# ronghanghu/vit_10b_fsdp_example

Hardware: AMD Instinct MI355X
Metric: images/sec (whole node) for ViT-10B bs=128 224px --fake_data (higher is better)
Workload: dtype bf16; 1 GPU; model=ViT-10B (5120d/32h/32L, patch14, 224px), global_batch=128, seq_len=256, parallelism=fsdp1, grad_ckpt=True, grad_ckpt_blocks=13, fuse_residual=False, init=device

## Files before the change

csrc/fgemm.hip:

```cpp

#ifndef VITFSDP_KERNELS_ONLY
#include <ATen/cuda/CUDAContext.h>
#include <torch/extension.h>

#include <cstdlib>
#endif

#include "mfma_tiles.h"

namespace {

constexpr int kBM = 256;
constexpr int kBN = 256;
constexpr int kThreads = 512;

template <int BK>
struct FgemmShared {
  static constexpr int SK = BK == 64 ? 64 : BK + 8;
  short a_tile[2][kBM][SK];
  short b_tile[2][kBN][SK];
};

template <int BK>
__device__ __forceinline__ int swz(int row, int col) {
  if (BK == 64) {
    return col ^ ((row & 7) * 8);
  }
  return col ^ (((row >> 3) & 1) * (BK / 2));
}

__device__ __forceinline__ bf16x8 lds_read_b128(unsigned byte_addr) {
  bf16x8 v;
  asm volatile("ds_read_b128 %0, %1 offset:0" : "=v"(v) : "v"(byte_addr));
  return v;
}

template <int EPI, int BK>
__global__ __launch_bounds__(kThreads, BK == 64 ? 1 : 2) void fgemm_abt_kernel(
    const short* __restrict__ a,
    const short* __restrict__ b,
    const short* __restrict__ bias,
    short* __restrict__ c,
    short* __restrict__ aux,
    int M, int N, int K) {
  constexpr bool WITH_BIAS = EPI >= 1;
  constexpr int kSK = FgemmShared<BK>::SK;
  constexpr int kChunks = BK / 32;
  HIP_DYNAMIC_SHARED(char, smem_raw)
  FgemmShared<BK>& sm = *reinterpret_cast<FgemmShared<BK>*>(smem_raw);

  const int tid = threadIdx.x;
  const int lane = tid & 63;
  const int wave = tid >> 6;
  const int col = lane & 15;
  const int seg = lane >> 4;
  const int wm = wave >> 2;
  const int wn = wave & 3;

  int bx = blockIdx.x, by = blockIdx.y;
  {
    const int gx = gridDim.x, gy = gridDim.y;
    const int nwg = gx * gy;
    const int bid = (int)(blockIdx.x + blockIdx.y * gx);
    int sx = 2, sy = 4;
    if (gy % 4 != 0) {
      if (gy % 2 == 0) { sx = 4; sy = 2; }
      else { sx = 8; sy = 1; }
    }
    if ((nwg & 7) == 0 && gx % sx == 0 && gy % sy == 0) {
      const int xcd = bid & 7, cid = bid >> 3;
      const int lw = gx / sx, lh = gy / sy;
      const int gm = (lw % 4 == 0) ? 4 : ((lw % 2 == 0) ? 2 : 1);
      const int per_band = gm * lh;
      const int band = cid / per_band, r = cid % per_band;
      bx = (xcd % sx) * lw + band * gm + (r % gm);
      by = (xcd / sx) * lh + r / gm;
    } else if ((nwg & 7) == 0) {
      const int swz = xcd_swizzle_m_major(bid, nwg);
      bx = swz % gx;
      by = swz / gx;
    }
  }
  const long m0 = (long)bx * kBM;
  const long n0 = (long)by * kBN;

  constexpr int kVecs = kBM * BK / 8 / kThreads;
  constexpr int kPerRow = BK / 8;
  const int s_r0 = tid / kPerRow;
  const int s_c8 = (tid % kPerRow) * 8;
  constexpr int kRowsPerCall = 1024 / (BK * 2);
  constexpr int kCalls = kBM / (8 * kRowsPerCall);
  bf16x8 a_st[BK == 64 ? 1 : kVecs], b_st[BK == 64 ? 1 : kVecs];
  auto issue_dtl = [&](int buf, long k_base) {
    const int l = lane;
    const int rsub = l >> 3;
#pragma unroll
    for (int i = 0; i < kCalls; ++i) {
      const int R = (wave * kCalls + i) * kRowsPerCall;
      const int row = R + rsub;
      const int g = (l & 7) ^ (row & 7);
      __builtin_amdgcn_global_load_lds(
          (const __attribute__((address_space(1))) void*)(
              &a[(m0 + row) * K + k_base + g * 8]),
          (__attribute__((address_space(3))) void*)&sm.a_tile[buf][R][0], 16,
          0, 0);
      __builtin_amdgcn_global_load_lds(
          (const __attribute__((address_space(1))) void*)(
              &b[(n0 + row) * K + k_base + g * 8]),
          (__attribute__((address_space(3))) void*)&sm.b_tile[buf][R][0], 16,
          0, 0);
    }
  };
  auto issue_loads = [&](long k_base) {
    if (BK == 64) return;
#pragma unroll
    for (int i = 0; i < kVecs && BK != 64; ++i) {
      const long row = s_r0 + i * (kThreads / kPerRow);
      a_st[i] =
          *reinterpret_cast<const bf16x8*>(&a[(m0 + row) * K + k_base + s_c8]);
      b_st[i] =
          *reinterpret_cast<const bf16x8*>(&b[(n0 + row) * K + k_base + s_c8]);
    }
  };
  auto write_tiles = [&](int buf) {
    if (BK == 64) return;
#pragma unroll
    for (int i = 0; i < kVecs && BK != 64; ++i) {
      const int row = s_r0 + i * (kThreads / kPerRow);
      const int cc = swz<BK>(row, s_c8);
      *reinterpret_cast<bf16x8*>(&sm.a_tile[buf][row][cc]) = a_st[i];
      *reinterpret_cast<bf16x8*>(&sm.b_tile[buf][row][cc]) = b_st[i];
    }
  };

  f32x4 acc[8][4];
#pragma unroll
  for (int mi = 0; mi < 8; ++mi)
#pragma unroll
    for (int ni = 0; ni < 4; ++ni) acc[mi][ni] = f32x4{0.f, 0.f, 0.f, 0.f};

  const int n_ksteps = K / BK;
  if (BK == 64) {
    issue_dtl(0, 0);
    asm volatile("s_waitcnt vmcnt(0)" ::: "memory");
  } else {
    issue_loads(0);
    write_tiles(0);
  }
  __syncthreads();

  const unsigned lds0 = (unsigned)__builtin_amdgcn_groupstaticsize();
  const unsigned a_base0 = lds0;
  const unsigned b_base0 = lds0 + (unsigned)sizeof(sm.a_tile);
  constexpr unsigned kABufBytes = sizeof(sm.a_tile[0]);
  constexpr unsigned kBBufBytes = sizeof(sm.b_tile[0]);

  for (int ks = 0; ks < n_ksteps; ++ks) {
    const int buf = ks & 1;
    const unsigned a_base = a_base0 + (unsigned)buf * kABufBytes;
    const unsigned b_base = b_base0 + (unsigned)buf * kBBufBytes;
#pragma unroll
    for (int kc = 0; kc < kChunks; ++kc) {
      if (BK == 64) {
        if (kc == 0 && ks + 1 < n_ksteps) issue_dtl(buf ^ 1, (long)(ks + 1) * BK);
      } else if (kc == kChunks - 1 && ks + 1 < n_ksteps) {
        issue_loads((long)(ks + 1) * BK);
      }
      const int kcol = kc * 32 + seg * 8;
      bf16x8 bf[4];
#pragma unroll
      for (int ni = 0; ni < 4; ++ni) {
        const int br = wn * 64 + ni * 16 + col;
        bf[ni] = lds_read_b128(
            b_base + 2u * ((unsigned)(br * kSK + swz<BK>(br, kcol))));
      }
      bf16x8 af[8];
#pragma unroll
      for (int mi = 0; mi < 8; ++mi) {
        const int ar = wm * 128 + mi * 16 + col;
        af[mi] = lds_read_b128(
            a_base + 2u * ((unsigned)(ar * kSK + swz<BK>(ar, kcol))));
      }
      asm volatile("s_waitcnt lgkmcnt(0)"
                   : "+v"(af[0]), "+v"(af[1]), "+v"(af[2]), "+v"(af[3]),
                     "+v"(af[4]), "+v"(af[5]), "+v"(af[6]), "+v"(af[7]),
                     "+v"(bf[0]), "+v"(bf[1]), "+v"(bf[2]), "+v"(bf[3])
                   :
                   : "memory");
      __builtin_amdgcn_s_setprio(1);
#pragma unroll
      for (int mi = 0; mi < 8; ++mi) {
#pragma unroll
        for (int ni = 0; ni < 4; ++ni) {
          acc[mi][ni] = __builtin_amdgcn_mfma_f32_16x16x32_bf16(
              af[mi], bf[ni], acc[mi][ni], 0, 0, 0);
        }
      }
      __builtin_amdgcn_s_setprio(0);
    }
    if (BK == 64) {
      if (ks + 1 < n_ksteps)
        asm volatile("s_waitcnt vmcnt(0)" ::: "memory");
    } else if (ks + 1 < n_ksteps) {
      write_tiles(buf ^ 1);
    }
    __syncthreads();
  }

  float bias_v[4];
  if (WITH_BIAS) {
#pragma unroll
    for (int ni = 0; ni < 4; ++ni) {
      bias_v[ni] = bf16_to_f32(
          (unsigned short)bias[n0 + wn * 64 + ni * 16 + col]);
    }
  }
#pragma unroll
  for (int mi = 0; mi < 8; ++mi) {
#pragma unroll
    for (int r = 0; r < 4; ++r) {
      const long m = m0 + wm * 128 + mi * 16 + seg * 4 + r;
#pragma unroll
      for (int ni = 0; ni < 4; ++ni) {
        const long n = n0 + wn * 64 + ni * 16 + col;
        float v = acc[mi][ni][r];
        if (WITH_BIAS) v += bias_v[ni];
        if (EPI == 2) {
          aux[m * N + n] = (short)f32_to_bf16(v);
          v = 0.5f * v * (1.f + erff(v * 0.70710678118654752f));
        }
        c[m * N + n] = (short)f32_to_bf16(v);
      }
    }
  }
}

template <int EPI>
__global__ __launch_bounds__(kThreads, 1) void fgemm_abt_mi32_kernel(
    const short* __restrict__ a, const short* __restrict__ b,
    const short* __restrict__ bias, short* __restrict__ c,
    short* __restrict__ aux, int M, int N, int K) {
  constexpr bool WITH_BIAS = EPI >= 1;
  constexpr int BK = 64;
  HIP_DYNAMIC_SHARED(char, smem_raw)
  FgemmShared<BK>& sm = *reinterpret_cast<FgemmShared<BK>*>(smem_raw);

  const int tid = threadIdx.x;
  const int lane = tid & 63;
  const int wave = tid >> 6;
  const int l31 = lane & 31;
  const int kseg = lane >> 5;
  const int wm = wave >> 2;
  const int wn = wave & 3;

  int bx = blockIdx.x, by = blockIdx.y;
  {
    const int gx = gridDim.x, gy = gridDim.y;
    const int nwg = gx * gy;
    const int bid = (int)(blockIdx.x + blockIdx.y * gx);
    int sx = 2, sy = 4;
    if (gy % 4 != 0) {
      if (gy % 2 == 0) { sx = 4; sy = 2; }
      else { sx = 8; sy = 1; }
    }
    if ((nwg & 7) == 0 && gx % sx == 0 && gy % sy == 0) {
      const int xcd = bid & 7, cid = bid >> 3;
      const int lw = gx / sx, lh = gy / sy;
      const int gm = (lw % 4 == 0) ? 4 : ((lw % 2 == 0) ? 2 : 1);
      const int per_band = gm * lh;
      const int band = cid / per_band, r = cid % per_band;
      bx = (xcd % sx) * lw + band * gm + (r % gm);
      by = (xcd / sx) * lh + r / gm;
    } else if ((nwg & 7) == 0) {
      const int swzb = xcd_swizzle_m_major(bid, nwg);
      bx = swzb % gx;
      by = swzb / gx;
    }
  }
  const long m0 = (long)bx * kBM;
  const long n0 = (long)by * kBN;

  auto issue_dtl = [&](int buf, long k_base) {
    const int rsub = lane >> 3;
#pragma unroll
    for (int i = 0; i < 4; ++i) {
      const int R = (wave * 4 + i) * 8;
      const int row = R + rsub;
      const int g = (lane & 7) ^ (row & 7);
      __builtin_amdgcn_global_load_lds(
          (const __attribute__((address_space(1))) void*)(
              &a[(m0 + row) * K + k_base + g * 8]),
          (__attribute__((address_space(3))) void*)&sm.a_tile[buf][R][0], 16,
          0, 0);
      __builtin_amdgcn_global_load_lds(
          (const __attribute__((address_space(1))) void*)(
              &b[(n0 + row) * K + k_base + g * 8]),
          (__attribute__((address_space(3))) void*)&sm.b_tile[buf][R][0], 16,
          0, 0);
    }
  };

  f32x16 acc[4][2];
#pragma unroll
  for (int mi = 0; mi < 4; ++mi)
#pragma unroll
    for (int ni = 0; ni < 2; ++ni) acc[mi][ni] = f32x16{};

  const int n_ksteps = K / BK;
  issue_dtl(0, 0);
  asm volatile("s_waitcnt vmcnt(0)" ::: "memory");
  __syncthreads();

  for (int ks = 0; ks < n_ksteps; ++ks) {
    const int buf = ks & 1;
    if (ks + 1 < n_ksteps) issue_dtl(buf ^ 1, (long)(ks + 1) * BK);
#pragma unroll
    for (int kc = 0; kc < 4; ++kc) {
      const int kcol = kc * 16 + kseg * 8;
      bf16x8 bf[2];
#pragma unroll
      for (int ni = 0; ni < 2; ++ni) {
        const int br = wn * 64 + ni * 32 + l31;
        bf[ni] = *reinterpret_cast<const bf16x8*>(
            &sm.b_tile[buf][br][swz<BK>(br, kcol)]);
      }
      __builtin_amdgcn_s_setprio(1);
#pragma unroll
      for (int mi = 0; mi < 4; ++mi) {
        const int ar = wm * 128 + mi * 32 + l31;
        const bf16x8 af = *reinterpret_cast<const bf16x8*>(
            &sm.a_tile[buf][ar][swz<BK>(ar, kcol)]);
#pragma unroll
        for (int ni = 0; ni < 2; ++ni) {
          acc[mi][ni] = __builtin_amdgcn_mfma_f32_32x32x16_bf16(
              af, bf[ni], acc[mi][ni], 0, 0, 0);
        }
      }
      __builtin_amdgcn_s_setprio(0);
    }
    if (ks + 1 < n_ksteps)
      asm volatile("s_waitcnt vmcnt(0)" ::: "memory");
    __syncthreads();
  }

  float bias_v[2];
  if (WITH_BIAS) {
#pragma unroll
    for (int ni = 0; ni < 2; ++ni) {
      bias_v[ni] = bf16_to_f32(
          (unsigned short)bias[n0 + wn * 64 + ni * 32 + l31]);
    }
  }
#pragma unroll
  for (int mi = 0; mi < 4; ++mi) {
#pragma unroll
    for (int g = 0; g < 4; ++g) {
#pragma unroll
      for (int r = 0; r < 4; ++r) {
        const long m = m0 + wm * 128 + mi * 32 + kseg * 4 + g * 8 + r;
#pragma unroll
        for (int ni = 0; ni < 2; ++ni) {
          const long n = n0 + wn * 64 + ni * 32 + l31;
          float v = acc[mi][ni][g * 4 + r];
          if (WITH_BIAS) v += bias_v[ni];
          if (EPI == 2) {
            aux[m * N + n] = (short)f32_to_bf16(v);
            v = 0.5f * v * (1.f + erff(v * 0.70710678118654752f));
          }
          c[m * N + n] = (short)f32_to_bf16(v);
        }
      }
    }
  }
}

#ifdef VITFSDP_KERNELS_ONLY
template __global__ void fgemm_abt_kernel<0, 64>(const short*, const short*,
                                                 const short*, short*, short*,
                                                 int, int, int);
template __global__ void fgemm_abt_kernel<1, 64>(const short*, const short*,
                                                 const short*, short*, short*,
                                                 int, int, int);
template __global__ void fgemm_abt_kernel<2, 64>(const short*, const short*,
                                                 const short*, short*, short*,
                                                 int, int, int);
template __global__ void fgemm_abt_kernel<0, 32>(const short*, const short*,
                                                 const short*, short*, short*,
                                                 int, int, int);
template __global__ void fgemm_abt_mi32_kernel<0>(const short*, const short*,
                                                  const short*, short*,
                                                  short*, int, int, int);
#endif

}

#ifndef VITFSDP_KERNELS_ONLY
namespace {

int fgemm_bk() {
  static int bk = [] {
    const char* e = std::getenv("VITFSDP_FGEMM_BK");
    return (e != nullptr && std::atoi(e) == 32) ? 32 : 64;
  }();
  return bk;
}

int fgemm_mi() {
  static int mi = [] {
    const char* e = std::getenv("VITFSDP_FGEMM_MI");
    return (e != nullptr && std::atoi(e) == 32) ? 32 : 16;
  }();
  return mi;
}

template <int EPI, int BK>
void launch_fgemm(const short* x, const short* w, const short* bias, short* c,
                  short* aux, long M, long N, long K, hipStream_t stream) {
  static bool attr_set = [] {
    (void)hipFuncSetAttribute(
        reinterpret_cast<const void*>(&fgemm_abt_kernel<EPI, BK>),
        hipFuncAttributeMaxDynamicSharedMemorySize, sizeof(FgemmShared<BK>));
    return true;
  }();
  (void)attr_set;
  dim3 grid((unsigned)(M / kBM), (unsigned)(N / kBN));
  hipLaunchKernelGGL((fgemm_abt_kernel<EPI, BK>), grid, dim3(kThreads),
                     sizeof(FgemmShared<BK>), stream, x, w, bias, c, aux,
                     (int)M, (int)N, (int)K);
}

template <int EPI>
void launch_fgemm_mi32(const short* x, const short* w, const short* bias,
                       short* c, short* aux, long M, long N, long K,
                       hipStream_t stream) {
  static bool attr_set = [] {
    (void)hipFuncSetAttribute(
        reinterpret_cast<const void*>(&fgemm_abt_mi32_kernel<EPI>),
        hipFuncAttributeMaxDynamicSharedMemorySize, sizeof(FgemmShared<64>));
    return true;
  }();
  (void)attr_set;
  dim3 grid((unsigned)(M / kBM), (unsigned)(N / kBN));
  hipLaunchKernelGGL((fgemm_abt_mi32_kernel<EPI>), grid, dim3(kThreads),
                     sizeof(FgemmShared<64>), stream, x, w, bias, c, aux,
                     (int)M, (int)N, (int)K);
}

template <int EPI>
void launch_fgemm_bk(const short* x, const short* w, const short* bias,
                     short* c, short* aux, long M, long N, long K,
                     hipStream_t stream) {
  if (fgemm_bk() == 32 && K % 32 == 0)
    launch_fgemm<EPI, 32>(x, w, bias, c, aux, M, N, K, stream);
  else if (fgemm_mi() == 32)
    launch_fgemm_mi32<EPI>(x, w, bias, c, aux, M, N, K, stream);
  else
    launch_fgemm<EPI, 64>(x, w, bias, c, aux, M, N, K, stream);
}

}

torch::Tensor fwd_gemm(torch::Tensor x, torch::Tensor w,
                       c10::optional<torch::Tensor> bias) {
  TORCH_CHECK(x.is_cuda() && x.is_contiguous() && w.is_contiguous(),
              "fwd_gemm: contiguous CUDA tensors required");
  TORCH_CHECK(x.scalar_type() == torch::kBFloat16 &&
              w.scalar_type() == torch::kBFloat16, "fwd_gemm: bf16 only");
  TORCH_CHECK(x.dim() == 2 && w.dim() == 2 && x.size(1) == w.size(1),
              "fwd_gemm: x[M,K], w[N,K] expected");
  const long M = x.size(0), K = x.size(1), N = w.size(0);
  TORCH_CHECK(M % kBM == 0 && N % kBN == 0 && K % 64 == 0,
              "fwd_gemm: needs M%256==0, N%256==0, K%64==0 (got ", M, ",", N,
              ",", K, ")");
  auto c = torch::empty({M, N}, x.options());
  const short* bias_ptr = nullptr;
  torch::Tensor bias_c;
  if (bias.has_value()) {
    bias_c = bias->contiguous();
    TORCH_CHECK(bias_c.scalar_type() == torch::kBFloat16 &&
                bias_c.numel() == N, "fwd_gemm: bias must be bf16 [N]");
    bias_ptr = (const short*)bias_c.data_ptr();
  }
  auto stream = at::cuda::getCurrentCUDAStream();
  if (bias_ptr) {
    launch_fgemm_bk<1>((const short*)x.data_ptr(), (const short*)w.data_ptr(),
                       bias_ptr, (short*)c.data_ptr(), nullptr, M, N, K,
                       stream);
  } else {
    launch_fgemm_bk<0>((const short*)x.data_ptr(), (const short*)w.data_ptr(),
                       nullptr, (short*)c.data_ptr(), nullptr, M, N, K,
                       stream);
  }
  HIP_CHECK_LAST();
  return c;
}

std::vector<torch::Tensor> fwd_gemm_gelu(torch::Tensor x, torch::Tensor w,
                                         torch::Tensor bias) {
  TORCH_CHECK(x.is_cuda() && x.is_contiguous() && w.is_contiguous() &&
              bias.is_contiguous(), "fwd_gemm_gelu: contiguous CUDA only");
  TORCH_CHECK(x.scalar_type() == torch::kBFloat16 &&
              w.scalar_type() == torch::kBFloat16 &&
              bias.scalar_type() == torch::kBFloat16,
              "fwd_gemm_gelu: bf16 only");
  TORCH_CHECK(x.dim() == 2 && w.dim() == 2 && x.size(1) == w.size(1) &&
              bias.numel() == w.size(0), "fwd_gemm_gelu: x[M,K], w[N,K]");
  const long M = x.size(0), K = x.size(1), N = w.size(0);
  TORCH_CHECK(M % kBM == 0 && N % kBN == 0 && K % 64 == 0,
              "fwd_gemm_gelu: needs M%256==0, N%256==0, K%64==0");
  auto c = torch::empty({M, N}, x.options());
  auto aux = torch::empty({M, N}, x.options());
  auto stream = at::cuda::getCurrentCUDAStream();
  launch_fgemm_bk<2>((const short*)x.data_ptr(), (const short*)w.data_ptr(),
                     (const short*)bias.data_ptr(), (short*)c.data_ptr(),
                     (short*)aux.data_ptr(), M, N, K, stream);
  HIP_CHECK_LAST();
  return {c, aux};
}
#endif
```

csrc/mfma_tiles.h:

```cpp
#pragma once

#include "common.h"

typedef __attribute__((ext_vector_type(8))) short bf16x8;
typedef __attribute__((ext_vector_type(4))) float f32x4;
typedef __attribute__((ext_vector_type(16))) float f32x16;
typedef __attribute__((ext_vector_type(2))) unsigned int u32x2;


__device__ __forceinline__ u32x2 tr16_read(unsigned lds_byte_addr) {
  u32x2 v;
  asm volatile("ds_read_b64_tr_b16 %0, %1 offset:0"
               : "=v"(v)
               : "v"(lds_byte_addr));
  return v;
}

template <int N>
__device__ __forceinline__ void lds_wait(u32x2& lo, u32x2& hi) {
  asm volatile("s_waitcnt lgkmcnt(%[cnt])"
               : "+v"(lo), "+v"(hi)
               : [cnt] "i"(N)
               : "memory");
}

__device__ __forceinline__ bf16x8 frag_from(u32x2 lo, u32x2 hi) {
  union {
    u32x2 uu[2];
    bf16x8 v;
  } cv;
  cv.uu[0] = lo;
  cv.uu[1] = hi;
  return cv.v;
}

__device__ __forceinline__ unsigned pack_bf16x2(float lo, float hi) {
  return (unsigned)f32_to_bf16(lo) | ((unsigned)f32_to_bf16(hi) << 16);
}

template <int NC, int STRIDE>
__device__ __forceinline__ void mfma_tr_ring(bf16x8 a, unsigned lds_base,
                                             int seg, int col,
                                             f32x4 (&acc)[NC]) {
  const unsigned lane_base =
      lds_base +
      2u * (unsigned)((seg * 8 + (col >> 2)) * STRIDE + (col & 3) * 4);
  u32x2 bf[2][2];
#pragma unroll
  for (int h = 0; h < 2; ++h)
    bf[0][h] = tr16_read(lane_base + 2u * (4 * h * STRIDE));
#pragma unroll
  for (int c = 0; c < NC; ++c) {
    const int cur = c & 1;
    if (c + 1 < NC) {
#pragma unroll
      for (int h = 0; h < 2; ++h)
        bf[cur ^ 1][h] =
            tr16_read(lane_base + 2u * (4 * h * STRIDE + (c + 1) * 16));
      lds_wait<2>(bf[cur][0], bf[cur][1]);
    } else {
      lds_wait<0>(bf[cur][0], bf[cur][1]);
    }
    acc[c] = __builtin_amdgcn_mfma_f32_16x16x32_bf16(
        a, frag_from(bf[cur][0], bf[cur][1]), acc[c], 0, 0, 0);
  }
}

__device__ __forceinline__ bf16x8 c_to_a_layout(const unsigned (&pk)[2][2],
                                                int seg, int col) {
  union {
    unsigned u[4];
    bf16x8 v;
  } cvt;
#pragma unroll
  for (int j2 = 0; j2 < 4; ++j2) {
    const int src = col + 16 * ((seg & 1) * 2 + (j2 >> 1));
    const unsigned lo = (unsigned)__shfl((int)pk[0][j2 & 1], src);
    const unsigned hi = (unsigned)__shfl((int)pk[1][j2 & 1], src);
    cvt.u[j2] = (seg >> 1) ? hi : lo;
  }
  return cvt.v;
}

template <int NKC, int D>
__device__ __forceinline__ void load_row_frags(const short* __restrict__ p,
                                               bool valid, int seg,
                                               bf16x8 (&frag)[NKC]) {
#pragma unroll
  for (int kc = 0; kc < NKC; ++kc) {
    const int d0 = kc * 32 + seg * 8;
    if (valid && d0 + 8 <= D) {
      frag[kc] = *reinterpret_cast<const bf16x8*>(&p[d0]);
    } else {
#pragma unroll
      for (int j = 0; j < 8; ++j)
        frag[kc][j] = (valid && d0 + j < D) ? p[d0 + j] : (short)0;
    }
  }
}

template <int ROWS, int COLS, int D, int THREADS>
struct TileStage {
  static constexpr int VPR = COLS / 8;
  static constexpr int N = (ROWS * VPR + THREADS - 1) / THREADS;
  int r[N], c[N];
  __device__ __forceinline__ TileStage() {
#pragma unroll
    for (int i = 0; i < N; ++i) {
      const int idx = (int)threadIdx.x + i * THREADS;
      r[i] = idx / VPR;
      c[i] = (idx % VPR) * 8;
    }
  }
  template <int M>
  __device__ __forceinline__ void load(const short* __restrict__ p,
                                       long row_stride, int row0, int T,
                                       bf16x8 (&st)[M]) const {
#pragma unroll
    for (int i = 0; i < N; ++i) {
      bf16x8 val = {0, 0, 0, 0, 0, 0, 0, 0};
      const int row = row0 + r[i];
      if (r[i] < ROWS && row < T && (COLS <= D || c[i] < D)) {
        val = *reinterpret_cast<const bf16x8*>(
            &p[(long)row * row_stride + c[i]]);
      }
      st[i] = val;
    }
  }
  template <int STRIDE, int M>
  __device__ __forceinline__ void store(short (*tile)[STRIDE],
                                        const bf16x8 (&st)[M]) const {
#pragma unroll
    for (int i = 0; i < N; ++i) {
      if (r[i] < ROWS) {
        *reinterpret_cast<bf16x8*>(&tile[r[i]][c[i]]) = st[i];
      }
    }
  }
};

__device__ __forceinline__ int xcd_swizzle_m_major(int bid, int nwg) {
  return (bid & 7) * (nwg >> 3) + (bid >> 3);
}
```

csrc/wgemm.hip:

```cpp

#ifndef VITFSDP_KERNELS_ONLY
#include <ATen/cuda/CUDAContext.h>
#include <torch/extension.h>
#endif

#include "mfma_tiles.h"

namespace {

constexpr int kBM = 256;
constexpr int kBN = 256;
constexpr int kBK = 64;
constexpr int kThreads = 512;
constexpr int kSA = kBM + 16;
constexpr int kSB = kBN + 16;

struct WgemmShared {
  short a_tile[2][kBK][kSA];
  short b_tile[2][kBK][kSB];
};

__device__ __forceinline__ u32x2 tr_read(unsigned lds_byte_base, int lane15,
                                         int row_base, int col_base,
                                         int row_stride) {
  return tr16_read(lds_byte_base +
                   2u * ((unsigned)((row_base + (lane15 >> 2)) * row_stride +
                                    col_base + (lane15 & 3) * 4)));
}

template <bool WITH_BIAS>
__global__ __launch_bounds__(kThreads, 2) void wgemm_atb_kernel(
    const short* __restrict__ a,
    const short* __restrict__ b,
    short* __restrict__ c,
    float* __restrict__ dbias,
    int K, int M, int N) {
  HIP_DYNAMIC_SHARED(char, smem_raw)
  WgemmShared& sm = *reinterpret_cast<WgemmShared*>(smem_raw);
  const unsigned a_base0 = (unsigned)__builtin_amdgcn_groupstaticsize();
  const unsigned b_base0 = a_base0 + sizeof(sm.a_tile);
  constexpr unsigned kABufBytes = sizeof(sm.a_tile[0]);
  constexpr unsigned kBBufBytes = sizeof(sm.b_tile[0]);

  const int tid = threadIdx.x;
  const int lane = tid & 63;
  const int wave = tid >> 6;
  const int col = lane & 15;
  const int seg = lane >> 4;
  const int wm = wave >> 2;
  const int wn = wave & 3;

  int bx = blockIdx.x, by = blockIdx.y;
  {
    const int nwg = gridDim.x * gridDim.y;
    if ((nwg & 7) == 0) {
      const int swz = xcd_swizzle_m_major(
          (int)(blockIdx.x + blockIdx.y * gridDim.x), nwg);
      bx = swz % gridDim.x;
      by = swz / gridDim.x;
    }
  }
  const long m0 = (long)bx * kBM;
  const long n0 = (long)by * kBN;

  constexpr int kVecs = kBK * (kBM / 8) / kThreads;
  const int s_kr0 = tid >> 5;
  const int s_c8 = (tid & 31) * 8;
  bf16x8 a_st[kVecs], b_st[kVecs];
  auto issue_loads = [&](long k_base) {
#pragma unroll
    for (int i = 0; i < kVecs; ++i) {
      const long krow = k_base + s_kr0 + i * 16;
      a_st[i] = *reinterpret_cast<const bf16x8*>(&a[krow * M + m0 + s_c8]);
      b_st[i] = *reinterpret_cast<const bf16x8*>(&b[krow * N + n0 + s_c8]);
    }
  };
  auto write_tiles = [&](int buf) {
#pragma unroll
    for (int i = 0; i < kVecs; ++i) {
      const int kr = s_kr0 + i * 16;
      *reinterpret_cast<bf16x8*>(&sm.a_tile[buf][kr][s_c8]) = a_st[i];
      *reinterpret_cast<bf16x8*>(&sm.b_tile[buf][kr][s_c8]) = b_st[i];
    }
  };

  f32x4 acc[8][4];
#pragma unroll
  for (int mi = 0; mi < 8; ++mi)
#pragma unroll
    for (int ni = 0; ni < 4; ++ni) acc[mi][ni] = f32x4{0.f, 0.f, 0.f, 0.f};

  float bias_acc[WITH_BIAS ? 8 : 1];
#pragma unroll
  for (int mi = 0; mi < (WITH_BIAS ? 8 : 1); ++mi) bias_acc[mi] = 0.f;

  const int n_ksteps = K / kBK;
  issue_loads(0);
  write_tiles(0);
  __syncthreads();

  for (int ks = 0; ks < n_ksteps; ++ks) {
    const int buf = ks & 1;
    const unsigned a_base = a_base0 + (unsigned)buf * kABufBytes;
    const unsigned b_base = b_base0 + (unsigned)buf * kBBufBytes;
#pragma unroll
    for (int kc = 0; kc < 2; ++kc) {
      if (kc == 1 && ks + 1 < n_ksteps) issue_loads((long)(ks + 1) * kBK);
      u32x2 bf[4][2];
#pragma unroll
      for (int ni = 0; ni < 4; ++ni) {
#pragma unroll
        for (int h = 0; h < 2; ++h) {
          bf[ni][h] = tr_read(b_base, col, kc * 32 + seg * 8 + 4 * h,
                              wn * 64 + ni * 16, kSB);
        }
      }
      u32x2 af[2][2];
#pragma unroll
      for (int h = 0; h < 2; ++h) {
        af[0][h] = tr_read(a_base, col, kc * 32 + seg * 8 + 4 * h,
                           wm * 128 + 0 * 16, kSA);
      }
#pragma unroll
      for (int mi = 0; mi < 8; ++mi) {
        const int cur = mi & 1;
        if (mi < 7) {
#pragma unroll
          for (int h = 0; h < 2; ++h) {
            af[cur ^ 1][h] =
                tr_read(a_base, col, kc * 32 + seg * 8 + 4 * h,
                        wm * 128 + (mi + 1) * 16, kSA);
          }
        }
        if (mi == 0) {
          asm volatile("s_waitcnt lgkmcnt(%[cnt])"
                       : "+v"(af[cur][0]), "+v"(af[cur][1]),
                         "+v"(bf[0][0]), "+v"(bf[0][1]), "+v"(bf[1][0]),
                         "+v"(bf[1][1]), "+v"(bf[2][0]), "+v"(bf[2][1])
                       : [cnt] "i"(2)
                       : "memory");
          asm volatile("" : "+v"(bf[3][0]), "+v"(bf[3][1]));
        } else if (mi < 7) {
          lds_wait<2>(af[cur][0], af[cur][1]);
        } else {
          lds_wait<0>(af[cur][0], af[cur][1]);
        }
        const bf16x8 a_frag = frag_from(af[cur][0], af[cur][1]);
        __builtin_amdgcn_s_setprio(1);
#pragma unroll
        for (int ni = 0; ni < 4; ++ni) {
          acc[mi][ni] = __builtin_amdgcn_mfma_f32_16x16x32_bf16(
              a_frag, frag_from(bf[ni][0], bf[ni][1]), acc[mi][ni], 0, 0, 0);
        }
        __builtin_amdgcn_s_setprio(0);
        if (WITH_BIAS && wn == 0) {
#pragma unroll
          for (int h = 0; h < 2; ++h) {
            bias_acc[mi] +=
                bf16_to_f32((unsigned short)(af[cur][h][0] & 0xffff)) +
                bf16_to_f32((unsigned short)(af[cur][h][0] >> 16)) +
                bf16_to_f32((unsigned short)(af[cur][h][1] & 0xffff)) +
                bf16_to_f32((unsigned short)(af[cur][h][1] >> 16));
          }
        }
      }
    }

    if (ks + 1 < n_ksteps) write_tiles(buf ^ 1);
    __syncthreads();
  }

#pragma unroll
  for (int mi = 0; mi < 8; ++mi) {
#pragma unroll
    for (int r = 0; r < 4; ++r) {
      const long m = m0 + wm * 128 + mi * 16 + seg * 4 + r;
#pragma unroll
      for (int ni = 0; ni < 4; ++ni) {
        const long n = n0 + wn * 64 + ni * 16 + col;
        c[m * N + n] = (short)f32_to_bf16(acc[mi][ni][r]);
      }
    }
    if (WITH_BIAS && wn == 0) {
      float v = bias_acc[mi];
      v += __shfl_xor(v, 16);
      v += __shfl_xor(v, 32);
      if (seg == 0) {
        atomicAdd(&dbias[m0 + wm * 128 + mi * 16 + col], v);
      }
    }
  }
}

#ifdef VITFSDP_KERNELS_ONLY
template __global__ void wgemm_atb_kernel<false>(const short*, const short*,
                                                 short*, float*, int, int,
                                                 int);
#endif

}

#ifndef VITFSDP_KERNELS_ONLY
std::vector<torch::Tensor> wgrad_gemm(torch::Tensor a, torch::Tensor b,
                                      bool with_bias) {
  TORCH_CHECK(a.is_cuda() && a.is_contiguous() && b.is_contiguous());
  TORCH_CHECK(a.scalar_type() == torch::kBFloat16 &&
              b.scalar_type() == torch::kBFloat16);
  TORCH_CHECK(a.dim() == 2 && b.dim() == 2 && a.size(0) == b.size(0));
  const long K = a.size(0), M = a.size(1), N = b.size(1);
  TORCH_CHECK(K % kBK == 0 && M % kBM == 0 && N % kBN == 0,
              "wgrad_gemm: needs K%64==0, M%256==0, N%256==0 (got ", K, ",",
              M, ",", N, ")");
  auto c = torch::empty({M, N}, a.options());
  torch::Tensor dbias;
  float* dbias_ptr = nullptr;
  if (with_bias) {
    dbias = torch::zeros({M}, a.options().dtype(torch::kFloat32));
    dbias_ptr = dbias.data_ptr<float>();
  }
  static bool attr_set = [] {
    hipFuncSetAttribute(
        reinterpret_cast<const void*>(&wgemm_atb_kernel<false>),
        hipFuncAttributeMaxDynamicSharedMemorySize, sizeof(WgemmShared));
    hipFuncSetAttribute(
        reinterpret_cast<const void*>(&wgemm_atb_kernel<true>),
        hipFuncAttributeMaxDynamicSharedMemorySize, sizeof(WgemmShared));
    return true;
  }();
  (void)attr_set;
  dim3 grid((unsigned)(M / kBM), (unsigned)(N / kBN));
  auto stream = at::cuda::getCurrentCUDAStream();
  if (with_bias) {
    hipLaunchKernelGGL(wgemm_atb_kernel<true>, grid, dim3(kThreads),
                       sizeof(WgemmShared), stream,
                       (const short*)a.data_ptr(), (const short*)b.data_ptr(),
                       (short*)c.data_ptr(), dbias_ptr, (int)K, (int)M,
                       (int)N);
  } else {
    hipLaunchKernelGGL(wgemm_atb_kernel<false>, grid, dim3(kThreads),
                       sizeof(WgemmShared), stream,
                       (const short*)a.data_ptr(), (const short*)b.data_ptr(),
                       (short*)c.data_ptr(), nullptr, (int)K, (int)M,
                       (int)N);
  }
  HIP_CHECK_LAST();
  if (with_bias) return {c, dbias};
  return {c};
}
#endif
```

vit_10b_fsdp_example_amd/ops/linear.py:

```python

import contextlib
import os

import torch
import torch.nn as nn
import torch.nn.functional as F
from torch.utils._python_dispatch import TorchDispatchMode

from ._extension import ext, use_hip
from ..tuning import lt_algo_table


_WGRAD_MODE = os.environ.get("VITFSDP_NATIVE_WGRAD", "0")
_NATIVE_WGRAD = _WGRAD_MODE == "1"
_NATIVE_WGRAD_DISPATCH = _WGRAD_MODE == "2"


def _use_native_wgrad(dy2, x2, w):
    if not _NATIVE_WGRAD:
        return False
    if not (dy2.is_cuda and dy2.dtype == torch.bfloat16):
        return False
    m, n = w.shape[0], w.shape[1]
    k = dy2.shape[0]
    if not (k % 64 == 0 and m % 256 == 0 and n % 256 == 0):
        return False
    if m > 16384 or n > 8192:
        return False
    return use_hip(dy2) and hasattr(ext(), "wgrad_gemm")


class _NativeLinearFn(torch.autograd.Function):
    @staticmethod
    def forward(ctx, x, weight, bias):
        ctx.save_for_backward(x, weight)
        ctx.has_bias = bias is not None
        return F.linear(x, weight, bias)

    @staticmethod
    def backward(ctx, dy):
        x, weight = ctx.saved_tensors
        dy2 = dy.reshape(-1, dy.shape[-1])
        x2 = x.reshape(-1, x.shape[-1])
        dx = torch.matmul(dy, weight)

        if _use_native_wgrad(dy2, x2, weight):
            (dw,) = ext().wgrad_gemm(dy2.contiguous(), x2.contiguous(), False)
            db = dy2.sum(0) if ctx.has_bias else None
        else:
            dw = torch.matmul(dy2.t(), x2)
            db = dy2.sum(0) if ctx.has_bias else None
        return dx, dw, db


_MIN_TILES = int(os.environ.get("VITFSDP_WGRAD_MIN_TILES", "256"))


def _wgrad_mm_shapes_ok(m, n, k):
    return (k % 64 == 0 and m % 256 == 0 and n % 256 == 0
            and m <= 16384 and n <= 16384
            and (m // 256) * (n // 256) >= _MIN_TILES)


def _is_wgrad_mm(at, b):
    if at.dim() != 2 or b.dim() != 2 or at.shape[1] != b.shape[0]:
        return False
    m, k = at.shape
    if m < 2 or k < 2:
        return False
    if not (at.stride(0) == 1 and at.stride(1) == m):
        return False
    if not (b.stride(1) == 1 and b.stride(0) == b.shape[1]):
        return False
    return _wgrad_mm_shapes_ok(m, b.shape[1], k)


class NativeWgradMode(TorchDispatchMode):

    def __init__(self, handler=None):
        super().__init__()
        self.hits = 0
        self._handler = handler

    def _route(self, at, b):
        if self._handler is not None:
            return self._handler(at.t(), b)
        (dw,) = ext().wgrad_gemm(at.t().contiguous(), b.contiguous(), False)
        return dw

    def __torch_dispatch__(self, func, types, args=(), kwargs=None):
        kwargs = kwargs or {}
        if (
            func is torch.ops.aten.mm.default
            and _is_wgrad_mm(*args)
            and (
                self._handler is not None
                or (
                    args[0].is_cuda
                    and args[0].dtype == torch.bfloat16
                    and args[1].dtype == torch.bfloat16
                    and use_hip(args[0])
                    and hasattr(ext(), "wgrad_gemm")
                )
            )
        ):
            self.hits += 1
            return self._route(*args)
        return func(*args, **kwargs)


def _op_layout(t):
    if t.dim() != 2:
        return None
    r, c = t.shape
    s0, s1 = t.stride()
    if s1 == 1 and (s0 == c or r == 1):
        return "N"
    if s0 == 1 and (s1 == r or c == 1):
        return "T"
    return None


def _dual_key(a, b):
    la, lb = _op_layout(a), _op_layout(b)
    if la is None or lb is None:
        return None
    return (lb, la, b.shape[1], a.shape[0], a.shape[1])



_GELU_CFG = {"d": 0, "hid": 0}

_FGEMM_MIN_TILES = int(os.environ.get("VITFSDP_FGEMM_MIN_TILES", "256"))


def configure_gelu_fusion(embed_dim, hidden_dim):
    if embed_dim != hidden_dim:
        _GELU_CFG["d"] = int(embed_dim)
        _GELU_CFG["hid"] = int(hidden_dim)


def _gelu_fusion_on():
    return (
        os.environ.get("VITFSDP_FUSED_GELU", "0") == "1"
        and _GELU_CFG["hid"] > 0
    )




def _dgelu_dbias_on():
    return (
        os.environ.get("VITFSDP_FUSED_DGELU_DBIAS", "1") != "0"
        and _GELU_CFG["hid"] > 0
    )



class TunedGemmMode(TorchDispatchMode):

    def __init__(self, table=None, native_wgrad=None, handler=None,
                 dgelu_handler=None):
        super().__init__()
        self.table = lt_algo_table() if table is None else table
        self.native_wgrad = (
            _NATIVE_WGRAD_DISPATCH if native_wgrad is None else native_wgrad
        )
        self._handler = handler
        self.hits = 0
        self.wgrad_hits = 0
        self.fused_gelu = _gelu_fusion_on()
        self._pending_gelu = {}
        self.gelu_hits = 0
        self._dgelu_handler = dgelu_handler
        self.fused_dgelu = _dgelu_dbias_on() and (
            dgelu_handler is not None or self._handler is None
        )
        self._dgelu_stash = None
        self.dgelu_hits = 0
        self.dbias_hits = 0

    def __exit__(self, exc_type, exc_val, exc_tb):
        self._dgelu_stash = None
        return super().__exit__(exc_type, exc_val, exc_tb)

    def _tuned_index(self, a, b):
        if not self.table:
            return None
        key = _dual_key(a, b)
        if key is None:
            return None
        return self.table.get(key)

    def _gpu_ok(self, t):
        if self._handler is not None:
            return True
        return t.is_cuda and t.dtype == torch.bfloat16 and use_hip(t)

    def _route(self, a, b, idx, bias=None):
        if self._handler is not None:
            return self._handler(a, b, idx, bias)
        return ext().lt_gemm(a, b, idx, bias)


    def _is_fc1_fwd(self, key):
        if not (
            key is not None
            and key[0] == "T" and key[1] == "N"
            and key[2] == _GELU_CFG["hid"] and key[4] == _GELU_CFG["d"]
        ):
            return False
        if self._handler is not None:
            return True
        hid, tok = key[2], key[3]
        return (
            tok % 256 == 0 and hid % 256 == 0 and key[4] % 64 == 0
            and (tok // 256) * (hid // 256) >= _FGEMM_MIN_TILES
        )

    def _fused_fc1_fwd(self, a, b, bias):
        if self._handler is not None:
            out, pre = self._handler(a, b, "gelu", bias)
        else:
            out, pre = ext().fwd_gemm_gelu(
                a.contiguous(), b.t().contiguous(), bias
            )
        self.gelu_hits += 1
        if len(self._pending_gelu) > 4:
            self._pending_gelu.clear()
        self._pending_gelu[pre.data_ptr()] = (pre, out)
        return pre


    def _is_mlp_dgelu(self, args, kwargs):
        if len(args) != 2 or kwargs.get("approximate", "none") != "none":
            return False
        dy, x = args
        if not (
            dy.dim() >= 2
            and dy.shape[-1] == _GELU_CFG["hid"]
            and dy.shape == x.shape
            and dy.is_contiguous() and x.is_contiguous()
        ):
            return False
        if self._dgelu_handler is not None:
            return True
        return (
            dy.is_cuda and dy.dtype == torch.bfloat16
            and x.dtype == torch.bfloat16
            and dy.shape[-1] % 8 == 0
            and use_hip(dy)
        )

    def _fused_dgelu(self, dy, x):
        if self._dgelu_handler is not None:
            dx, colsum = self._dgelu_handler(dy, x)
        else:
            dx, colsum = ext().gelu_bwd_colsum(dy, x)
        self.dgelu_hits += 1
        self._dgelu_stash = (dx, colsum)
        return dx

    def _stashed_dbias(self, args, kwargs):
        if self._dgelu_stash is None or kwargs.get("dtype") is not None:
            return None
        dx, colsum = self._dgelu_stash
        t = args[0]
        dims = args[1] if len(args) > 1 else None
        keepdim = args[2] if len(args) > 2 else kwargs.get("keepdim", False)
        if not (
            isinstance(t, torch.Tensor)
            and dims is not None
            and t.dtype == dx.dtype
            and t.device == dx.device
            and t.untyped_storage().data_ptr()
            == dx.untyped_storage().data_ptr()
            and t.storage_offset() == dx.storage_offset()
            and t.numel() == dx.numel()
            and t.dim() >= 2
            and t.shape[-1] == dx.shape[-1]
            and t.is_contiguous()
            and sorted(d % t.dim() for d in dims) == list(range(t.dim() - 1))
        ):
            return None
        self._dgelu_stash = None
        self.dbias_hits += 1
        if keepdim:
            return colsum.view([1] * (t.dim() - 1) + [t.shape[-1]])
        return colsum

    def __torch_dispatch__(self, func, types, args=(), kwargs=None):
        kwargs = kwargs or {}
        if func is torch.ops.aten.mm.default and self._gpu_ok(args[0]):
            a, b = args
            if (
                self.native_wgrad
                and self._handler is None
                and _is_wgrad_mm(a, b)
                and hasattr(ext(), "wgrad_gemm")
            ):
                self.wgrad_hits += 1
                (dw,) = ext().wgrad_gemm(a.t().contiguous(), b.contiguous(),
                                         False)
                return dw
            idx = self._tuned_index(a, b)
            if idx is not None:
                self.hits += 1
                return self._route(a, b, idx)
        elif (
            func is torch.ops.aten.addmm.default
            and len(args) == 3
            and kwargs.get("beta", 1) == 1
            and kwargs.get("alpha", 1) == 1
            and self._gpu_ok(args[1])
            and args[0].dim() == 1
        ):
            bias, a, b = args
            key = _dual_key(a, b)
            if (
                self.fused_gelu
                and self._is_fc1_fwd(key)
                and (self._handler is not None
                     or hasattr(ext(), "fwd_gemm_gelu"))
            ):
                return self._fused_fc1_fwd(a, b, bias)
            idx = self.table.get(key) if (self.table and key) else None
            if idx is not None:
                self.hits += 1
                return self._route(a, b, idx, bias)
        elif self.fused_gelu and func is torch.ops.aten.gelu.default:
            _, out = self._pending_gelu.pop(args[0].data_ptr(), (None, None))
            if out is not None and out.shape == args[0].shape:
                return out
        elif self.fused_dgelu and func is torch.ops.aten.gelu_backward.default:
            if self._is_mlp_dgelu(args, kwargs):
                return self._fused_dgelu(*args)
        elif (
            self._dgelu_stash is not None
            and func is torch.ops.aten.sum.dim_IntList
        ):
            out = self._stashed_dbias(args, kwargs)
            if out is not None:
                return out
        return func(*args, **kwargs)


def gemm_dispatch_context():
    if lt_algo_table() or _gelu_fusion_on() or _dgelu_dbias_on():
        return TunedGemmMode()
    if _NATIVE_WGRAD_DISPATCH:
        return NativeWgradMode()
    return contextlib.nullcontext()


def wgrad_backward_context():
    return gemm_dispatch_context()


class NativeLinear(nn.Linear):

    def forward(self, x):
        if _NATIVE_WGRAD:
            return _NativeLinearFn.apply(x, self.weight, self.bias)
        return F.linear(x, self.weight, self.bias)
```

Before: 65.60 images/sec.

## Rework wgrad GEMM with direct-to-LDS loads, XOR swizzle, and enable it by default

Rewrites the native weight-gradient GEMM so tiles are loaded straight from global memory into LDS via global_load_lds, replacing the register staging and LDS write-back. LDS tiles lose their padding and use an XOR chunk swizzle instead, with precomputed per-lane offsets and immediate-offset transposed reads. The kernel also adopts the shared XCD-clustered tile mapping, now factored into a helper, and launch bounds drop to one block per CU. The default VITFSDP_NATIVE_WGRAD mode becomes dispatch mode 2, so this kernel replaces the library wgrad path, which risks being slower than hipBLASLt for some shapes.

New measurement: 66.26 images/sec (median of 6 runs). +1.0%, better.

```diff
diff --git a/csrc/fgemm.hip b/csrc/fgemm.hip
--- a/csrc/fgemm.hip
+++ b/csrc/fgemm.hip
@@ -57,30 +57,8 @@
   const int wm = wave >> 2;
   const int wn = wave & 3;
 
-  int bx = blockIdx.x, by = blockIdx.y;
-  {
-    const int gx = gridDim.x, gy = gridDim.y;
-    const int nwg = gx * gy;
-    const int bid = (int)(blockIdx.x + blockIdx.y * gx);
-    int sx = 2, sy = 4;
-    if (gy % 4 != 0) {
-      if (gy % 2 == 0) { sx = 4; sy = 2; }
-      else { sx = 8; sy = 1; }
-    }
-    if ((nwg & 7) == 0 && gx % sx == 0 && gy % sy == 0) {
-      const int xcd = bid & 7, cid = bid >> 3;
-      const int lw = gx / sx, lh = gy / sy;
-      const int gm = (lw % 4 == 0) ? 4 : ((lw % 2 == 0) ? 2 : 1);
-      const int per_band = gm * lh;
-      const int band = cid / per_band, r = cid % per_band;
-      bx = (xcd % sx) * lw + band * gm + (r % gm);
-      by = (xcd / sx) * lh + r / gm;
-    } else if ((nwg & 7) == 0) {
-      const int swz = xcd_swizzle_m_major(bid, nwg);
-      bx = swz % gx;
-      by = swz / gx;
-    }
-  }
+  int bx, by;
+  xcd_cluster_tile(bx, by);
   const long m0 = (long)bx * kBM;
   const long n0 = (long)by * kBN;
 
@@ -253,30 +231,8 @@
   const int wm = wave >> 2;
   const int wn = wave & 3;
 
-  int bx = blockIdx.x, by = blockIdx.y;
-  {
-    const int gx = gridDim.x, gy = gridDim.y;
-    const int nwg = gx * gy;
-    const int bid = (int)(blockIdx.x + blockIdx.y * gx);
-    int sx = 2, sy = 4;
-    if (gy % 4 != 0) {
-      if (gy % 2 == 0) { sx = 4; sy = 2; }
-      else { sx = 8; sy = 1; }
-    }
-    if ((nwg & 7) == 0 && gx % sx == 0 && gy % sy == 0) {
-      const int xcd = bid & 7, cid = bid >> 3;
-      const int lw = gx / sx, lh = gy / sy;
-      const int gm = (lw % 4 == 0) ? 4 : ((lw % 2 == 0) ? 2 : 1);
-      const int per_band = gm * lh;
-      const int band = cid / per_band, r = cid % per_band;
-      bx = (xcd % sx) * lw + band * gm + (r % gm);
-      by = (xcd / sx) * lh + r / gm;
-    } else if ((nwg & 7) == 0) {
-      const int swzb = xcd_swizzle_m_major(bid, nwg);
-      bx = swzb % gx;
-      by = swzb / gx;
-    }
-  }
+  int bx, by;
+  xcd_cluster_tile(bx, by);
   const long m0 = (long)bx * kBM;
   const long n0 = (long)by * kBN;
 
diff --git a/csrc/mfma_tiles.h b/csrc/mfma_tiles.h
--- a/csrc/mfma_tiles.h
+++ b/csrc/mfma_tiles.h
@@ -13,6 +13,16 @@
   asm volatile("ds_read_b64_tr_b16 %0, %1 offset:0"
                : "=v"(v)
                : "v"(lds_byte_addr));
+  return v;
+}
+
+template <int OFF>
+__device__ __forceinline__ u32x2 tr16_read_at(unsigned lds_byte_addr) {
+  static_assert(OFF >= 0 && OFF < 65536, "ds offset field is 16 bits");
+  u32x2 v;
+  asm volatile("ds_read_b64_tr_b16 %0, %1 offset:%2"
+               : "=v"(v)
+               : "v"(lds_byte_addr), "n"(OFF));
   return v;
 }
 
@@ -142,3 +152,29 @@
 __device__ __forceinline__ int xcd_swizzle_m_major(int bid, int nwg) {
   return (bid & 7) * (nwg >> 3) + (bid >> 3);
 }
+
+__device__ __forceinline__ void xcd_cluster_tile(int& bx, int& by) {
+  bx = blockIdx.x;
+  by = blockIdx.y;
+  const int gx = gridDim.x, gy = gridDim.y;
+  const int nwg = gx * gy;
+  const int bid = (int)(blockIdx.x + blockIdx.y * gx);
+  int sx = 2, sy = 4;
+  if (gy % 4 != 0) {
+    if (gy % 2 == 0) { sx = 4; sy = 2; }
+    else { sx = 8; sy = 1; }
+  }
+  if ((nwg & 7) == 0 && gx % sx == 0 && gy % sy == 0) {
+    const int xcd = bid & 7, cid = bid >> 3;
+    const int lw = gx / sx, lh = gy / sy;
+    const int gm = (lw % 4 == 0) ? 4 : ((lw % 2 == 0) ? 2 : 1);
+    const int per_band = gm * lh;
+    const int band = cid / per_band, r = cid % per_band;
+    bx = (xcd % sx) * lw + band * gm + (r % gm);
+    by = (xcd / sx) * lh + r / gm;
+  } else if ((nwg & 7) == 0) {
+    const int swz = xcd_swizzle_m_major(bid, nwg);
+    bx = swz % gx;
+    by = swz / gx;
+  }
+}
diff --git a/csrc/wgemm.hip b/csrc/wgemm.hip
--- a/csrc/wgemm.hip
+++ b/csrc/wgemm.hip
@@ -12,24 +12,26 @@
 constexpr int kBN = 256;
 constexpr int kBK = 64;
 constexpr int kThreads = 512;
-constexpr int kSA = kBM + 16;
-constexpr int kSB = kBN + 16;
+static_assert(kBM == kBN, "one staging/read scheme serves both tiles");
+constexpr int kRowBytes = kBM * 2;
 
 struct WgemmShared {
-  short a_tile[2][kBK][kSA];
-  short b_tile[2][kBK][kSB];
+  short a_tile[2][kBK][kBM];
+  short b_tile[2][kBK][kBN];
 };
 
-__device__ __forceinline__ u32x2 tr_read(unsigned lds_byte_base, int lane15,
-                                         int row_base, int col_base,
-                                         int row_stride) {
-  return tr16_read(lds_byte_base +
-                   2u * ((unsigned)((row_base + (lane15 >> 2)) * row_stride +
-                                    col_base + (lane15 & 3) * 4)));
+__device__ __forceinline__ int chunk_xor(int k) {
+  return (k & 3) | (((k >> 3) & 1) << 2);
+}
+
+__device__ __forceinline__ void glds16(const short* gsrc, short* lds_dst) {
+  __builtin_amdgcn_global_load_lds(
+      (const __attribute__((address_space(1))) void*)gsrc,
+      (__attribute__((address_space(3))) void*)lds_dst, 16, 0, 0);
 }
 
 template <bool WITH_BIAS>
-__global__ __launch_bounds__(kThreads, 2) void wgemm_atb_kernel(
+__global__ __launch_bounds__(kThreads, 1) void wgemm_atb_kernel(
     const short* __restrict__ a,
     const short* __restrict__ b,
     short* __restrict__ c,
@@ -50,39 +52,35 @@
   const int wm = wave >> 2;
   const int wn = wave & 3;
 
-  int bx = blockIdx.x, by = blockIdx.y;
-  {
-    const int nwg = gridDim.x * gridDim.y;
-    if ((nwg & 7) == 0) {
-      const int swz = xcd_swizzle_m_major(
-          (int)(blockIdx.x + blockIdx.y * gridDim.x), nwg);
-      bx = swz % gridDim.x;
-      by = swz / gridDim.x;
-    }
-  }
+  int bx, by;
+  xcd_cluster_tile(bx, by);
   const long m0 = (long)bx * kBM;
   const long n0 = (long)by * kBN;
 
-  constexpr int kVecs = kBK * (kBM / 8) / kThreads;
-  const int s_kr0 = tid >> 5;
-  const int s_c8 = (tid & 31) * 8;
-  bf16x8 a_st[kVecs], b_st[kVecs];
-  auto issue_loads = [&](long k_base) {
-#pragma unroll
-    for (int i = 0; i < kVecs; ++i) {
-      const long krow = k_base + s_kr0 + i * 16;
-      a_st[i] = *reinterpret_cast<const bf16x8*>(&a[krow * M + m0 + s_c8]);
-      b_st[i] = *reinterpret_cast<const bf16x8*>(&b[krow * N + n0 + s_c8]);
+  constexpr int kCalls = kBK / 2 / (kThreads / 64);
+  auto issue_dtl = [&](int buf, long k_base) {
+    const int rsub = lane >> 5;
+    const int gl = lane & 31;
+#pragma unroll
+    for (int i = 0; i < kCalls; ++i) {
+      const int R = (wave * kCalls + i) * 2;
+      const int k = R + rsub;
+      const int g = (((gl >> 1) ^ chunk_xor(k)) << 1) | (gl & 1);
+      glds16(&a[(k_base + k) * M + m0 + g * 8], &sm.a_tile[buf][R][0]);
+      glds16(&b[(k_base + k) * N + n0 + g * 8], &sm.b_tile[buf][R][0]);
     }
   };
-  auto write_tiles = [&](int buf) {
-#pragma unroll
-    for (int i = 0; i < kVecs; ++i) {
-      const int kr = s_kr0 + i * 16;
-      *reinterpret_cast<bf16x8*>(&sm.a_tile[buf][kr][s_c8]) = a_st[i];
-      *reinterpret_cast<bf16x8*>(&sm.b_tile[buf][kr][s_c8]) = b_st[i];
-    }
-  };
+
+  const int xr = (col >> 2) | ((seg & 1) << 2);
+  const unsigned lane_off =
+      (unsigned)((seg * 8 + (col >> 2)) * kRowBytes + (col & 3) * 8);
+  unsigned a_off[8], b_off[4];
+#pragma unroll
+  for (int mi = 0; mi < 8; ++mi)
+    a_off[mi] = lane_off + ((unsigned)((wm * 8 + mi) ^ xr) << 5);
+#pragma unroll
+  for (int ni = 0; ni < 4; ++ni)
+    b_off[ni] = lane_off + ((unsigned)((wn * 4 + ni) ^ xr) << 5);
 
   f32x4 acc[8][4];
 #pragma unroll
@@ -95,43 +93,35 @@
   for (int mi = 0; mi < (WITH_BIAS ? 8 : 1); ++mi) bias_acc[mi] = 0.f;
 
   const int n_ksteps = K / kBK;
-  issue_loads(0);
-  write_tiles(0);
+  issue_dtl(0, 0);
+  asm volatile("s_waitcnt vmcnt(0)" ::: "memory");
   __syncthreads();
 
   for (int ks = 0; ks < n_ksteps; ++ks) {
     const int buf = ks & 1;
     const unsigned a_base = a_base0 + (unsigned)buf * kABufBytes;
     const unsigned b_base = b_base0 + (unsigned)buf * kBBufBytes;
+    if (ks + 1 < n_ksteps) issue_dtl(buf ^ 1, (long)(ks + 1) * kBK);
 #pragma unroll
     for (int kc = 0; kc < 2; ++kc) {
-      if (kc == 1 && ks + 1 < n_ksteps) issue_loads((long)(ks + 1) * kBK);
+      auto rd = [&](unsigned addr, u32x2 (&f)[2]) {
+        if (kc == 0) {
+          f[0] = tr16_read_at<0>(addr);
+          f[1] = tr16_read_at<4 * kRowBytes>(addr);
+        } else {
+          f[0] = tr16_read_at<32 * kRowBytes>(addr);
+          f[1] = tr16_read_at<36 * kRowBytes>(addr);
+        }
+      };
       u32x2 bf[4][2];
 #pragma unroll
-      for (int ni = 0; ni < 4; ++ni) {
-#pragma unroll
-        for (int h = 0; h < 2; ++h) {
-          bf[ni][h] = tr_read(b_base, col, kc * 32 + seg * 8 + 4 * h,
-                              wn * 64 + ni * 16, kSB);
-        }
-      }
+      for (int ni = 0; ni < 4; ++ni) rd(b_base + b_off[ni], bf[ni]);
       u32x2 af[2][2];
-#pragma unroll
-      for (int h = 0; h < 2; ++h) {
-        af[0][h] = tr_read(a_base, col, kc * 32 + seg * 8 + 4 * h,
-                           wm * 128 + 0 * 16, kSA);
-      }
+      rd(a_base + a_off[0], af[0]);
 #pragma unroll
       for (int mi = 0; mi < 8; ++mi) {
         const int cur = mi & 1;
-        if (mi < 7) {
-#pragma unroll
-          for (int h = 0; h < 2; ++h) {
-            af[cur ^ 1][h] =
-                tr_read(a_base, col, kc * 32 + seg * 8 + 4 * h,
-                        wm * 128 + (mi + 1) * 16, kSA);
-          }
-        }
+        if (mi < 7) rd(a_base + a_off[mi + 1], af[cur ^ 1]);
         if (mi == 0) {
           asm volatile("s_waitcnt lgkmcnt(%[cnt])"
                        : "+v"(af[cur][0]), "+v"(af[cur][1]),
@@ -166,7 +156,7 @@
       }
     }
 
-    if (ks + 1 < n_ksteps) write_tiles(buf ^ 1);
+    if (ks + 1 < n_ksteps) asm volatile("s_waitcnt vmcnt(0)" ::: "memory");
     __syncthreads();
   }
 
diff --git a/vit_10b_fsdp_example_amd/ops/linear.py b/vit_10b_fsdp_example_amd/ops/linear.py
--- a/vit_10b_fsdp_example_amd/ops/linear.py
+++ b/vit_10b_fsdp_example_amd/ops/linear.py
@@ -11,7 +11,7 @@
 from ..tuning import lt_algo_table
 
 
-_WGRAD_MODE = os.environ.get("VITFSDP_NATIVE_WGRAD", "0")
+_WGRAD_MODE = os.environ.get("VITFSDP_NATIVE_WGRAD", "2")
 _NATIVE_WGRAD = _WGRAD_MODE == "1"
 _NATIVE_WGRAD_DISPATCH = _WGRAD_MODE == "2"
 
```
